# openai/ot-gan

Hardware: AMD Instinct MI355X
Metric: OT-GAN train images/sec (CIFAR-10 32x32, bs=256/GPU) (higher is better)
Workload: dtype f32 (Winograd-domain GEMMs on the fp16 matrix pipe with operands split into two scaled fp16 pieces = 22 significand bits, fp32 accumulate; errors at or below the fp32 MFMA chain's)

## Files before the change

### include/otgan_layers.h

```cpp
#ifndef OTGAN_LAYERS_H
#define OTGAN_LAYERS_H

#define OTGAN_ACT_NONE 0
#define OTGAN_ACT_CRELU 1
#define OTGAN_ACT_CELU 2
#define OTGAN_ACT_ELU 3
#define OTGAN_ACT_RELU 4

typedef struct otgan_conv_desc {
  int N;
  int H, W;
  int C;
  int ldx;
  int upsample;
  int KH, KW;
  int stride;
  int Cout;
  int ldy;
  int y_coff;
  int preact;
  int list_quads;
  const float* x_amax;
  const float* dy_amax;
  int y_accumulate;
// ... 60 lines not shown
int otgan_conv2d_dgrad_pf_f32(const otgan_conv_desc* d, const float* dy, const float* w, const void* filters,
                              const float* x, const int32_t* inv, float* dx, int lddx,
                              int accumulate, void* workspace, size_t workspace_bytes, void* stream);

int otgan_conv2d_wgrad_f32(const otgan_conv_desc* d, const float* x, const int32_t* cmap,
                           const float* dy, float* dw, void* workspace, size_t workspace_bytes,
                           void* stream);

int otgan_weightnorm_fwd_f32(const float* V, const float* g, int K, int Cout, float* w,
                             float* wT, float* inv_norm, void* stream);
int otgan_weightnorm_fwd_amax_f32(const float* V, const float* g, int K, int Cout, float* w, float* wT,
                                  float* inv_norm, float* w_amax, void* stream);
int otgan_weightnorm_bwd_f32(const float* V, const float* g, const float* inv_norm,
                             const float* dw, int K, int Cout, float* dV, float* dg,
                             float* scratch, void* stream);

#define OTGAN_WN_MAX_LAYERS 16
typedef struct otgan_wn_fwd_layer {
  const float* V;
  const float* g;
  float* w;
  float* wT;
  float* inv;
  int K;
} otgan_wn_fwd_layer;
typedef struct otgan_wn_part {
  const float* p;
  const int32_t* perm;
  int nrows;
  int rstride;
// ... 28 lines not shown
int otgan_feature_head_bwd_amax_f32(const float* x, const float* f, const float* norm, const float* df, int N, int HW,
                                    int C, float* dx, float* dx_amax, void* stream);

int otgan_adam_step_f32(float* p, const float* grad, float* v, float* mg, long n, double lr,
                        double mom1, double mom2, double t, void* stream);
#define OTGAN_ADAM_MAX_SEGMENTS 32
int otgan_adam_step_gather_f32(float* p, const float* const* grads, const long* offsets, int nseg, float* v, float* mg,
                               double lr, double mom1, double mom2, double t, float* ema_shadow, double ema_decay,
                               void* stream);
void otgan_adam_coefficients(double mom1, double mom2, double t, float* out2);
int otgan_adam_step_coef_f32(float* p, const float* grad, float* v, float* mg, long n, double lr,
                             double mom1, double mom2, double t, const float* coef_dev, void* stream);
int otgan_adam_step_gather_coef_f32(float* p, const float* const* grads, const long* offsets, int nseg, float* v, float* mg,
                                    double lr, double mom1, double mom2, double t, const float* coef_dev, float* ema_shadow,
                                    double ema_decay, void* stream);
#define OTGAN_COPY2D_MAX_SEGMENTS 64
int otgan_copy2d_batched_f32(const float* const* src, float* const* dst, const int* rows, const int* cols,
                             const long* src_ld, const long* dst_ld, int nseg, void* stream);
#define OTGAN_GATHER3D_MAX_SEGMENTS 32
int otgan_gather3d_batched_f32(const float* const* src, float* const* dst, const int* n0, int n1, int n2,
                               const long* src_s0, const long* src_s1, const long* dst_s0, const long* dst_s1,
                               int base1, const int* map1_dev, float* amax_out, int nseg, void* stream);
int otgan_adamax_step_f32(float* p, const float* grad, float* v, float* mg, long n, double lr,
                          double mom1, double mom2, void* stream);
int otgan_nesterov_step_f32(float* p, const float* grad, float* v, long n, double lr, double mom1,
                            void* stream);
int otgan_ema_update_f32(float* shadow, const float* p, long n, double decay, void* stream);

typedef struct otgan_incep_conv_desc {
  int N, H, W;
// ... 40 lines not shown
```

### ot-gan_amd/_lib_layers.py

```python
import ctypes

c_fp = ctypes.c_void_p
c_int, c_long, c_float, c_size_t = ctypes.c_int, ctypes.c_long, ctypes.c_float, ctypes.c_size_t
c_double = ctypes.c_double


class ConvDesc(ctypes.Structure):
    _fields_ = [("N", c_int), ("H", c_int), ("W", c_int), ("C", c_int), ("ldx", c_int),
                ("upsample", c_int), ("KH", c_int), ("KW", c_int), ("stride", c_int),
                ("Cout", c_int), ("ldy", c_int), ("y_coff", c_int), ("preact", c_int),
                ("list_quads", c_int), ("x_amax", ctypes.c_void_p), ("dy_amax", ctypes.c_void_p),
                ("y_accumulate", c_int), ("x_operand", ctypes.c_void_p),
                ("y_amax_out", ctypes.c_void_p), ("dx_amax_out", ctypes.c_void_p), ("w_amax", ctypes.c_void_p),
                ("x_amax_count", c_int), ("list_width", c_int),
                ("glu_out", ctypes.c_void_p), ("glu_amax_out", ctypes.c_void_p), ("dy_amax_count", c_int)]


P_DESC = ctypes.POINTER(ConvDesc)


class IncepConvDesc(ctypes.Structure):
    _fields_ = [("N", c_int), ("H", c_int), ("W", c_int), ("C", c_int), ("ldx", c_int), ("KH", c_int), ("KW", c_int),
                ("stride_h", c_int), ("stride_w", c_int), ("same", c_int), ("Cout", c_int), ("ldy", c_int),
                ("y_coff", c_int), ("relu", c_int)]
# ... 5 lines not shown
                ("y_coff", c_int)]


INCEP_POOL_MAX, INCEP_POOL_AVG = 0, 1


class Dense16BwdPair(ctypes.Structure):
    _fields_ = [("w", ctypes.c_void_p), ("fwd_filters", ctypes.c_void_p), ("filters", ctypes.c_void_p),
                ("nslices_src", c_int), ("slice_index", c_int), ("pair_index", c_int)]


class WnFwdLayer(ctypes.Structure):
    _fields_ = [("V", c_fp), ("g", c_fp), ("w", c_fp), ("wT", c_fp), ("inv", c_fp), ("K", c_int)]


class WnPart(ctypes.Structure):
    _fields_ = [("p", c_fp), ("perm", c_fp), ("nrows", c_int), ("rstride", c_int)]


class WnBwdLayer(ctypes.Structure):
    _fields_ = [("V", c_fp), ("g", c_fp), ("inv", c_fp), ("dV", c_fp), ("dg", c_fp), ("Ceff", c_int), ("taps", c_int),
                ("part", WnPart * 3)]


SIGNATURES = {
    "otgan_conv2d_workspace_bytes": (c_size_t, [P_DESC, c_int]),
    "otgan_conv2d_operand_bytes": (c_size_t, [P_DESC]),
    "otgan_conv2d_glu_fused": (c_int, [P_DESC]),
    "otgan_absmax_f32": (c_int, [c_fp, c_long, c_int, c_long, c_fp, c_fp]),
    "otgan_conv2d_amax_fused": (c_int, [P_DESC, c_int]),
# ... 8 lines not shown
    "otgan_dense16_prepare_filters_f32": (c_int, [c_fp, c_fp, c_fp, c_int, c_fp]),
    "otgan_dense16_h2_ok": (c_int, [P_DESC]),
    "otgan_dense16_chain_fwd_f32": (c_int, [c_int, c_int, c_int, c_int, c_fp, c_int, c_fp, c_fp, c_fp]),
    "otgan_dense16_chain_bwd_f32": (c_int, [c_int, c_int, c_int, c_int, c_fp, c_int, c_fp, c_int, c_fp, c_fp, c_fp, c_fp]),
    "otgan_dense16_bwd_filter_bytes": (c_size_t, [c_int]),
    "otgan_dense16_prepare_bwd_filters_f32": (c_int, [c_fp, c_int, c_fp, c_int, c_fp]),
    "otgan_dense16_bwd_slice_f32": (c_int, [c_int, c_int, c_int, c_int, c_fp, c_int, c_fp, c_fp, c_int, c_fp, c_fp, c_int,
                                            c_fp, c_int, c_fp, c_fp]),
    "otgan_conv2d_prepare_filters_f32": (c_int, [P_DESC, c_int, c_fp, c_fp, c_size_t, c_fp]),
    "otgan_conv2d_fwd_pf_f32": (c_int, [P_DESC, c_fp, c_fp, c_fp, c_fp, c_fp, c_fp, c_fp, c_size_t, c_fp]),
    "otgan_conv2d_dgrad_pf_f32": (c_int, [P_DESC, c_fp, c_fp, c_fp, c_fp, c_fp, c_fp, c_int, c_int, c_fp,
                                          c_size_t, c_fp]),
    "otgan_weightnorm_fwd_f32": (c_int, [c_fp, c_fp, c_int, c_int, c_fp, c_fp, c_fp, c_fp]),
    "otgan_weightnorm_fwd_amax_f32": (c_int, [c_fp, c_fp, c_int, c_int, c_fp, c_fp, c_fp, c_fp, c_fp]),
    "otgan_weightnorm_bwd_f32": (c_int, [c_fp, c_fp, c_fp, c_fp, c_int, c_int, c_fp, c_fp, c_fp, c_fp]),
    "otgan_weightnorm_fwd_batched16_f32": (c_int, [ctypes.POINTER(WnFwdLayer), c_int, c_fp]),
    "otgan_weightnorm_bwd_batched16_f32": (c_int, [ctypes.POINTER(WnBwdLayer), c_int, c_fp]),
    "otgan_colsum_f32": (c_int, [c_fp, c_long, c_int, c_long, c_fp, c_fp, c_fp]),
    "otgan_glu_fwd_f32": (c_int, [c_fp, c_long, c_int, c_fp, c_fp]),
    "otgan_glu_bwd_f32": (c_int, [c_fp, c_fp, c_long, c_int, c_fp, c_fp]),
    "otgan_glu_fwd_amax_f32": (c_int, [c_fp, c_long, c_int, c_fp, c_fp, c_fp]),
    "otgan_glu_bwd_amax_f32": (c_int, [c_fp, c_fp, c_long, c_int, c_fp, c_fp, c_fp]),
    "otgan_feature_head_bwd_amax_f32": (c_int, [c_fp, c_fp, c_fp, c_fp, c_int, c_int, c_int, c_fp, c_fp, c_fp]),
    "otgan_tanh_fwd_f32": (c_int, [c_fp, c_long, c_fp, c_fp]),
    "otgan_tanh_bwd_f32": (c_int, [c_fp, c_fp, c_long, c_fp, c_fp]),
    "otgan_feature_head_fwd_f32": (c_int, [c_fp, c_int, c_int, c_int, c_fp, c_fp, c_fp]),
    "otgan_feature_head_bwd_f32": (c_int, [c_fp, c_fp, c_fp, c_fp, c_int, c_int, c_int, c_fp, c_fp]),
    "otgan_adam_step_f32": (c_int, [c_fp, c_fp, c_fp, c_fp, c_long, c_double, c_double, c_double,
                                    c_double, c_fp]),
    "otgan_adam_step_gather_f32": (c_int, [c_fp, c_fp, c_fp, c_int, c_fp, c_fp, c_double, c_double, c_double, c_double,
# ... 24 lines not shown
```

### ot-gan_amd/csrc/pointwise.hip

```cpp
#include "common.h"
#include "../../include/otgan.h"

namespace {

constexpr int kChunks = 256;

inline int grid_for(long n, int per_thread = 4) {
  long b = ceil_div_l(n, 256L * per_thread);
  if (b > 4096) b = 4096;
  if (b < 1) b = 1;
  return (int)b;
}

template <int OP>
__global__ __launch_bounds__(256) void colreduce_kernel(const float* __restrict__ a,
                                                        const float* __restrict__ b, long rows,
                                                        int cols, long lda,
                                                        float* __restrict__ partial) {
  const int lane = threadIdx.x & 63, wave = threadIdx.x >> 6;
  const int c = blockIdx.x * 64 + lane;
  const int chunk = blockIdx.y;
  const long per = ceil_div_l(rows, (long)gridDim.y);
  const long r0 = chunk * per;
  long r1 = r0 + per;
// ... 62 lines not shown
  __shared__ float4 red[16][17];
  red[rsub][cq] = s;
  __syncthreads();
  if (threadIdx.x < 16 && c < cols) {
    float4 t = make_float4(0.f, 0.f, 0.f, 0.f);
#pragma unroll
    for (int k = 0; k < 16; ++k) {
      const float4 v = red[k][threadIdx.x];
      t.x += v.x; t.y += v.y; t.z += v.z; t.w += v.w;
    }
    const int cc = blockIdx.x * 64 + 4 * threadIdx.x;
    *reinterpret_cast<float4*>(partial + (long)chunk * cols + cc) = t;
  }
}

template <int OP>
int colreduce(const float* a, const float* b, long rows, int cols, long lda, float* partial,
              int* nchunk_out, hipStream_t s) {
  const int colblocks = ceil_div(cols, 64);
  long nchunk = ceil_div(1024, colblocks);
  if (nchunk > kChunks) nchunk = kChunks;
  if (nchunk > ceil_div_l(rows, 64)) nchunk = ceil_div_l(rows, 64);
  if (nchunk < 1) nchunk = 1;
  dim3 grid(colblocks, (int)nchunk);
  const bool vec = (cols % 4 == 0) && (lda % 4 == 0) && ((reinterpret_cast<uintptr_t>(a) & 15) == 0) &&
                   (!b || (reinterpret_cast<uintptr_t>(b) & 15) == 0) &&
                   ((reinterpret_cast<uintptr_t>(partial) & 15) == 0);
  if (vec) hipLaunchKernelGGL(colreduce4_kernel<OP>, grid, dim3(256), 0, s, a, b, rows, cols, lda, partial);
  else hipLaunchKernelGGL(colreduce_kernel<OP>, grid, dim3(256), 0, s, a, b, rows, cols, lda, partial);
  *nchunk_out = (int)nchunk;
  OTGAN_CHECK_LAUNCH("colreduce");
  return OTGAN_OK;
}

__global__ __launch_bounds__(256) void weightnorm_apply_kernel(const float* __restrict__ V,
                                                               const float* __restrict__ g,
                                                               const float* __restrict__ inv,
                                                               int K, int Cout,
// ... 15 lines not shown
    tile[ty + 8 * i][tx] = v;
    const unsigned b = amax_bits(v);
    mb = b > mb ? b : mb;
  }
  if (wT) {
    __syncthreads();
#pragma unroll
    for (int i = 0; i < 4; ++i) {
      const int c = c0 + ty + 8 * i, k = k0 + tx;
      if (k < K && c < Cout) wT[(long)c * K + k] = tile[tx][ty + 8 * i];
    }
  }
  if (rec) amax_commit(rec, mb);
}

__global__ void weightnorm_bwd_kernel(const float* __restrict__ V, const float* __restrict__ g,
                                      const float* __restrict__ inv, const float* __restrict__ dw,
                                      const float* __restrict__ dot, long total, int Cout,
                                      float* __restrict__ dV) {
  for (long i = (long)blockIdx.x * blockDim.x + threadIdx.x; i < total;
       i += (long)gridDim.x * blockDim.x) {
    const int c = (int)(i % Cout);
    const float iv = inv[c];
    dV[i] = g[c] * iv * (dw[i] - V[i] * dot[c] * iv * iv);
  }
}
__global__ __launch_bounds__(256) void wn_dot_finish_kernel(const float* __restrict__ partial, int nchunk, int cols,
                                                            const float* __restrict__ inv, float* __restrict__ dot,
                                                            float* __restrict__ dg) {
  const int lane = threadIdx.x & 63, part = threadIdx.x >> 6;
  const int c = blockIdx.x * 64 + lane;
  float s = 0.f;
  if (c < cols)
    for (int k = part; k < nchunk; k += 4) s += partial[(long)k * cols + c];
  __shared__ float red[4][64];
  red[part][lane] = s;
  __syncthreads();
  if (part == 0 && c < cols) {
    const float t = (red[0][lane] + red[1][lane]) + (red[2][lane] + red[3][lane]);
    dot[c] = t;
    dg[c] = t * inv[c];
  }
}
__global__ void weightnorm_dg_kernel(const float* __restrict__ dot, const float* __restrict__ inv,
                                     int Cout, float* __restrict__ dg) {
  const int c = blockIdx.x * blockDim.x + threadIdx.x;
  if (c < Cout) dg[c] = dot[c] * inv[c];
}

constexpr int kWnThreads = 512, kWnRowLanes = kWnThreads / 4;
inline bool aligned16(const void* p) { return (reinterpret_cast<uintptr_t>(p) & 15) == 0; }
struct WnFwdArgs {
  otgan_wn_fwd_layer l[OTGAN_WN_MAX_LAYERS];
};
struct WnBwdArgs {
  otgan_wn_bwd_layer l[OTGAN_WN_MAX_LAYERS];
// ... 487 lines not shown
                                   float* __restrict__ sh, float decay, float omd, const float* __restrict__ coef) {
  if (coef) {
    c1 = coef[0];
    c2 = coef[1];
  }
  const int seg = blockIdx.y;
  const long base = segs.off[seg], n = segs.off[seg + 1] - base;
  const float* __restrict__ g = segs.g[seg];
  for (long i = (long)blockIdx.x * blockDim.x + threadIdx.x; i < n; i += (long)gridDim.x * blockDim.x) {
    const long j = base + i;
    const float pn = adam_elem(p[j], g[i], v, mg, j, lr, mom1, om1, mom2, om2, c1, c2);
    p[j] = pn;
    if (sh) sh[j] = ema_elem(sh[j], pn, decay, omd);
  }
}
__global__ void ema_kernel(float* __restrict__ sh, const float* __restrict__ p, long n, float decay,
                           float omd) {
  for (long i = (long)blockIdx.x * blockDim.x + threadIdx.x; i < n; i += (long)gridDim.x * blockDim.x)
    sh[i] = ema_elem(sh[i], p[i], decay, omd);
}

}

extern "C" {

int otgan_weightnorm_fwd_amax_f32(const float* V, const float* g, int K, int Cout, float* w, float* wT,
                                  float* inv_norm, float* w_amax, void* stream) {
  OTGAN_CHECK_ARG(V && g && w && inv_norm && K > 0 && Cout > 0, "bad arguments");
  hipStream_t s = (hipStream_t)stream;
  ProfScope ps(OTGAN_PROF_POINTWISE, 0.0, 4.0 * 3 * (double)K * Cout, s);
// ... 10 lines not shown
}
int otgan_weightnorm_fwd_f32(const float* V, const float* g, int K, int Cout, float* w, float* wT, float* inv_norm,
                             void* stream) {
  return otgan_weightnorm_fwd_amax_f32(V, g, K, Cout, w, wT, inv_norm, nullptr, stream);
}

int otgan_weightnorm_bwd_f32(const float* V, const float* g, const float* inv_norm, const float* dw,
                             int K, int Cout, float* dV, float* dg, float* scratch, void* stream) {
  OTGAN_CHECK_ARG(V && g && inv_norm && dw && dV && dg && scratch && K > 0 && Cout > 0, "bad arguments");
  hipStream_t s = (hipStream_t)stream;
  ProfScope ps(OTGAN_PROF_POINTWISE, 0.0, 4.0 * 5 * (double)K * Cout, s);
  float* partial = dV;
  int nchunk = 0;
  int rc = colreduce<2>(dw, V, K, Cout, Cout, partial, &nchunk, s);
  if (rc) return rc;
  hipLaunchKernelGGL(wn_dot_finish_kernel, dim3(ceil_div(Cout, 64)), dim3(256), 0, s, partial, nchunk, Cout, inv_norm, scratch, dg);
  const long total = (long)K * Cout;
  hipLaunchKernelGGL(weightnorm_bwd_kernel, dim3(grid_for(total)), dim3(256), 0, s, V, g, inv_norm, dw,
                     scratch, total, Cout, dV);
  OTGAN_CHECK_LAUNCH("weightnorm bwd");
  return OTGAN_OK;
}

int otgan_weightnorm_fwd_batched16_f32(const otgan_wn_fwd_layer* layers, int n_layers, void* stream) {
  OTGAN_CHECK_ARG(layers && n_layers > 0, "bad arguments");
  hipStream_t s = (hipStream_t)stream;
  double bytes = 0.0;
  for (int i = 0; i < n_layers; ++i) {
    const otgan_wn_fwd_layer& l = layers[i];
    OTGAN_CHECK_ARG(l.V && l.g && l.w && l.inv && l.K > 0, "layer %d: null pointer or empty", i);
    OTGAN_CHECK_ARG(aligned16(l.V) && aligned16(l.g) && aligned16(l.w) && aligned16(l.inv), "layer %d: 16-byte alignment", i);
    bytes += 4.0 * 4 * (double)l.K * 16;
  }
  ProfScope ps(OTGAN_PROF_POINTWISE, 0.0, bytes, s);
  for (int i0 = 0; i0 < n_layers; i0 += OTGAN_WN_MAX_LAYERS) {
// ... 182 lines not shown
    segs.g[i] = grads[i];
    segs.off[i] = offsets[i];
    if (offsets[i + 1] - offsets[i] > longest) longest = offsets[i + 1] - offsets[i];
  }
  segs.off[nseg] = offsets[nseg];
  const long n = offsets[nseg] - offsets[0];
  ProfScope ps(OTGAN_PROF_POINTWISE, 0.0, 4.0 * (ema_shadow ? 9 : 7) * (double)n, s);
  float c[2] = {1.f, 1.f};
  if (!coef_dev) otgan_adam_coefficients(mom1, mom2, t, c);
  hipLaunchKernelGGL(adam_gather_kernel, dim3(grid_for(longest), nseg), dim3(256), 0, s, p, segs, v, mg, (float)lr,
                     (float)mom1, (float)(1.0 - mom1), (float)mom2, (float)(1.0 - mom2), c[0], c[1], ema_shadow,
                     (float)ema_decay, (float)(1.0 - ema_decay), coef_dev);
  OTGAN_CHECK_LAUNCH("adam (gathered gradients)");
  return OTGAN_OK;
}
int otgan_adamax_step_f32(float* p, const float* grad, float* v, float* mg, long n, double lr,
                          double mom1, double mom2, void* stream) {
  OTGAN_CHECK_ARG(p && grad && mg && n > 0 && (mom1 <= 0.0 || v), "bad arguments");
  hipLaunchKernelGGL(adamax_kernel, dim3(grid_for(n)), dim3(256), 0, (hipStream_t)stream, p, grad, v,
                     mg, n, (float)lr, (float)mom1, (float)(1.0 - mom1), (float)mom2);
  OTGAN_CHECK_LAUNCH("adamax");
  return OTGAN_OK;
}
int otgan_nesterov_step_f32(float* p, const float* grad, float* v, long n, double lr, double mom1,
                            void* stream) {
  OTGAN_CHECK_ARG(p && grad && v && n > 0, "bad arguments");
  hipLaunchKernelGGL(nesterov_kernel, dim3(grid_for(n)), dim3(256), 0, (hipStream_t)stream, p, grad,
                     v, n, (float)lr, (float)mom1, (float)(1.0 + mom1));
  OTGAN_CHECK_LAUNCH("nesterov");
  return OTGAN_OK;
// ... 11 lines not shown
```

### ot-gan_amd/ops.py

```python
import ctypes
import os
import sys
import weakref
from collections import OrderedDict

import torch

from . import _lib
from ._lib_layers import ConvDesc, WnBwdLayer, WnFwdLayer

ACT = {None: 0, "none": 0, "crelu": 1, "celu": 2, "elu": 3, "relu": 4}
DOUBLED = (1, 2)

_ws = {}


class _NullCtx:
    def __enter__(self):
        return None

    def __exit__(self, *exc):
        return False


# ... 149 lines not shown
    return w, wT, inv


def weightnorm_bwd(V2d, g, inv, dw):
    K, Cout = V2d.shape
    dV = torch.empty_like(V2d)
    dg = torch.empty_like(g)
    scratch = torch.empty(Cout, dtype=V2d.dtype, device=V2d.device)
    _lib.check(_lib.lib().otgan_weightnorm_bwd_f32(V2d.data_ptr(), g.data_ptr(), inv.data_ptr(),
                                                   dw.data_ptr(), K, Cout, dV.data_ptr(),
                                                   dg.data_ptr(), scratch.data_ptr(),
                                                   _lib.stream_ptr()), "weightnorm_bwd")
    return dV, dg


def colsum(a2d_ptr, rows, cols, lda, device):
    out = torch.empty(cols, dtype=torch.float32, device=device)
    scratch = torch.empty(256 * cols, dtype=torch.float32, device=device)
    _lib.check(_lib.lib().otgan_colsum_f32(a2d_ptr, rows, cols, lda, out.data_ptr(),
                                           scratch.data_ptr(), _lib.stream_ptr()), "colsum")
    return out


_LAUNCH_POINTERS = ("x_amax", "dy_amax", "w_amax", "y_amax_out", "dx_amax_out", "glu_out", "glu_amax_out", "x_operand")
_LAUNCH_INTS = ("ldy", "y_accumulate")


def launch_desc(desc, **fields):
    d = ConvDesc.from_buffer_copy(desc)
    for name, v in fields.items():
# ... 162 lines not shown
                                        dy.data_ptr(), dw.data_ptr(), ws.data_ptr(), ws.numel(),
                                        _lib.stream_ptr()), "conv2d_wgrad")


def fold_weights(desc, w):
    nfold = _lib.lib().otgan_conv2d_folded_weight_elems(ctypes.byref(desc))
    weff = torch.empty(nfold, dtype=w.dtype, device=w.device)
    weffT = torch.empty(nfold, dtype=w.dtype, device=w.device)
    _lib.check(_lib.lib().otgan_conv2d_fold_weights_f32(ctypes.byref(desc), w.data_ptr(), weff.data_ptr(),
                                                        weffT.data_ptr(), _lib.stream_ptr()), "fold_weights")
    return weff, weffT


SIDE_STREAM = None
_SIDE_SEEN = set()


def join_side_stream(tensors=()):
    _SIDE_SEEN.clear()
    if SIDE_STREAM is None:
        return
    cur = torch.cuda.current_stream()
    cur.wait_stream(SIDE_STREAM)
    for t in tensors:
        if t is not None and t.is_cuda:
            t.record_stream(cur)


_PENDING_GLU = [None]


def _drop_unclaimed_glu():
    ref = _PENDING_GLU[0]
    if ref is not None:
        t = ref()
        if t is not None:
            take(t, "glu", remove=True)
        _PENDING_GLU[0] = None


SIGN_TRACE = None
# ... 114 lines not shown
            conv_dgrad_raw(desc, dy, w, x, ctx.inv, dx, x.shape[3], False, filt["bwd"], dx_amax_out=dx_rec)
            if dx_rec is not None:
                tag_amax(dx, dx_rec)
        need_w = ctx.needs_input_grad[1] or ctx.needs_input_grad[2]
        need_b = ctx.has_b and ctx.needs_input_grad[3]
        side = SIDE_STREAM if (need_w or need_b) else None
        if side is not None:
            side.wait_stream(torch.cuda.current_stream())
            for t in (dy, x, ctx.x_op, dy_rec, ctx.x_rec):
                if t is not None:
                    t.record_stream(side)
        with (torch.cuda.stream(side) if side is not None else _NULL_CTX):
            if need_w:
                dw = torch.empty_like(V2d)
                conv_wgrad_raw(desc, x, ctx.cmap, dy, dw)
                dV2d, dg = weightnorm_bwd(V2d, g, inv_norm, dw)
                dV = dV2d.view(ctx.vshape)
            if need_b:
                db = colsum_of(dy)
                if db is None:
                    rows = dy.numel() // dy.shape[-1]
                    db = colsum(dy.data_ptr(), rows, dy.shape[-1], ld, dy.device)
        if side is not None:
            key = V2d.untyped_storage().data_ptr() + V2d.storage_offset()
            if key in _SIDE_SEEN:
                torch.cuda.current_stream().wait_stream(side)
            _SIDE_SEEN.add(key)
        return dx, dV, dg, db, None, None, None, None, None, None


def conv2d_op(x, V, g, b, stride=1, upsample=False, preact=0, segs=None, glu_hint=False, grow=0):
    return Conv2dFunction.apply(x, V, g, b, int(stride), bool(upsample), int(preact),
# ... 821 lines not shown


def adam_coefficients(mom1, mom2, t):
    out = (ctypes.c_float * 2)()
    _lib.lib().otgan_adam_coefficients(float(mom1), float(mom2), float(t), ctypes.cast(out, ctypes.c_void_p))
    return float(out[0]), float(out[1])


def adam_step_gather(p_flat, grads, offsets, v, mg, lr, mom1, mom2, t, ema_shadow=None, ema_decay=0.0, coef=None):
    n = len(grads)
    bump_weights_epoch(p_flat)
    if ema_shadow is not None:
        bump_weights_epoch(ema_shadow)
    gp = (ctypes.c_void_p * n)(*[g.data_ptr() for g in grads])
    off = (ctypes.c_long * (n + 1))(*offsets)
    _lib.check(_lib.lib().otgan_adam_step_gather_coef_f32(p_flat.data_ptr(), ctypes.cast(gp, ctypes.c_void_p),
                                                          ctypes.cast(off, ctypes.c_void_p), n, _lib.ptr(v), mg.data_ptr(),
                                                          float(lr), float(mom1), float(mom2), float(t), _lib.ptr(coef),
                                                          _lib.ptr(ema_shadow), float(ema_decay), _lib.stream_ptr()),
               "adam_step_gather")


COPY2D_MAX_SEGMENTS = 64


def copy2d_batched(segs):
    for i0 in range(0, len(segs), COPY2D_MAX_SEGMENTS):
        part = segs[i0:i0 + COPY2D_MAX_SEGMENTS]
        n = len(part)
        src = (ctypes.c_void_p * n)(*[q[0] for q in part])
# ... 82 lines not shown
```

### ot-gan_amd/trainer.py

```python
import importlib
import os

import torch

from . import parallel
from .utils import matching, nn


def _lib_prof_on():
    from . import _lib
    return _lib.prof_enabled()


class _frozen:

    def __init__(self, params):
        self.params = [p for p in params if p.requires_grad]

    def __enter__(self):
        for p in self.params:
            p.requires_grad_(False)

    def __exit__(self, *exc):
        for p in self.params:
# ... 95 lines not shown
        overlap = self.collectives and self.collectives_mode == "overlapped"
        self.disc_buckets = parallel.GradBuckets(self.disc_params) if overlap else None
        self.gen_buckets = parallel.GradBuckets(self.gen_params) if overlap else None
        self.gen_optimizer = mk[args.optimizer](self.gen_params, **kw)
        self.disc_optimizer = mk[args.optimizer](self.disc_params, **kw)
        self.ema_fused = self.gen_optimizer.fuse_ema(self.ema)
        self.step_counter = 0
        self.last = {}
        import collections
        self._max_ahead = 2
        self._step_ends, self._free_events = collections.deque(), []
        self.timers = None
        self._d_weights_in_graph = False
        on = side_ok
        self.fork_real_pass = self.fork_wgrad = on
        self._side_stream = torch.cuda.Stream(device=device) if on else None
        env = os.environ.get("OTGAN_STEP_GRAPH")
        asked = getattr(args, "step_graph", None)
        want = (env == "1") if env in ("0", "1") else (args.model == "densenet" if asked is None else bool(asked))
        self.graphs = GraphedSteps(self) if (want and not self.collectives and self.world == 1) else None

    def enable_timers(self, on=True):
        self.timers = {} if on else None
        if on and self.graphs is not None:
            self.graphs.drop("region timers need the eager step")
            self.graphs = None

    def _timed(self, name):
        if self.timers is None:
            return _NO_REGION
# ... 81 lines not shown

    def step(self, x_data, noise=None, apply_updates=True):
        assert x_data.shape[0] == self.nb
        period = self.args.nr_gen_per_disc + 1
        phase = self.step_counter % period
        kind = "disc" if phase == 0 else "gen"
        self._throttle()
        if self.graphs is not None and noise is None and apply_updates:
            done = self.graphs.run(x_data, phase)
            if done is not None:
                self.last = done
                self._mark_step_end()
                return self.last
        from . import ops
        ops.SIDE_STREAM = self._side_stream if self.fork_wgrad else None
        try:
            dist, ent, grads = self._step_body(x_data, kind, noise, apply_updates)
        finally:
            ops.SIDE_STREAM = None
        self._mark_step_end()
        self._d_weights_in_graph = False
        self.step_counter += 1
        self.last = {"kind": kind, "distance": dist, "entropy": ent}
        if not apply_updates:
            self.last["grads"] = grads
        return self.last

    def _throttle(self):
        if self._max_ahead > 0 and len(self._step_ends) >= self._max_ahead:
            ev = self._step_ends.popleft()
            ev.synchronize()
            self._free_events.append(ev)

    def _mark_step_end(self):
        if self._max_ahead > 0:
            ev = self._free_events.pop() if self._free_events else torch.cuda.Event()
            ev.record()
            self._step_ends.append(ev)
            if len(self._step_ends) > self._max_ahead:
                self._free_events.append(self._step_ends.popleft())

    def _optimise(self, opt, grads, lr, critic):
        opt(grads, lr=lr)
        if not critic and not self.ema_fused:
            self.maintain_averages()

    def _backward(self, outputs, params, grad_outputs):
        from . import ops
        grads = torch.autograd.grad(outputs, params, grad_outputs)
        if self.fork_wgrad:
            ops.join_side_stream(grads)
        return grads

    def prepare_step_graphs(self, x_data):
        if self.graphs is None:
            return 0
        period = self.args.nr_gen_per_disc + 1
        kinds = {self.graphs._kind(p) for p in range(period)}
        n = 0
        while self.graphs is not None and self.graphs.dead is None and set(self.graphs.graphs) != kinds and n < 3 * period + 2:
            self.step(x_data)
            n += 1
        return n
# ... 205 lines not shown
            if hasattr(opt, "ensure_state"):
                opt.ensure_state()
                if opt.coef_dev is None:
                    opt.coef_dev = torch.ones(2, dtype=torch.float32, device=m.device)
        self.x.copy_(x_data)
        ts = list(m.gen_params) + [m.ema.average(p) for p in m.gen_params]
        if kind == "gen1":
            ts += list(m.disc_params)
        self._bump(ts)
        saved_t = (m.gen_optimizer.t, m.disc_optimizer.t)
        ops.reset_amax_pool()
        g = torch.cuda.CUDAGraph()
        try:
            m.gen_optimizer.capturing = m.disc_optimizer.capturing = True
            ops.SIDE_STREAM = m._side_stream if m.fork_wgrad else None
            with torch.cuda.graph(g, stream=self.stream):
                try:
                    dist, ent, _ = m._step_body(self.x, "disc" if kind == "disc" else "gen")
                except BaseException:
                    if ops.SIDE_STREAM is not None:
                        torch.cuda.current_stream().wait_stream(ops.SIDE_STREAM)
                    raise
        finally:
            ops.SIDE_STREAM = None
            m.gen_optimizer.capturing = m.disc_optimizer.capturing = False
            m.gen_optimizer.t, m.disc_optimizer.t = saved_t
            ops.reset_amax_pool()
            ops.forget_side_events()
        self.graphs[kind] = (g, dist, ent)
        if kind == "gen1":
            self.critic_ops = ops.weights_in(m.disc_params[0])


def rank_log_kernel_slices(rank, world, f_gen, f_dat, fa, fb, lam):
    def halves(f):
        if torch.is_tensor(f):
            return f[:f.shape[0] // 2], f[f.shape[0] // 2:]
        return torch.cat(f[:len(f) // 2], 0), torch.cat(f[len(f) // 2:], 0)
    a2 = halves(fa)[1]
# ... 77 lines not shown
```

### ot-gan_amd/utils/nn.py

```python
import contextlib
import os
import threading
import weakref
from collections import OrderedDict

import torch

from .. import ops

_scope = threading.local()


def _stack():
    if not hasattr(_scope, "stack"):
        _scope.stack = []
    return _scope.stack


@contextlib.contextmanager
def arg_scope(funcs, **kwargs):
    _stack().append(({f.__name__ for f in funcs}, kwargs))
    try:
        yield
    finally:
# ... 337 lines not shown
    def __init__(self, params, lr, mom1, mom2):
        self.params = list(params)
        self.lr, self.mom1, self.mom2 = lr, mom1, mom2
        self.group = FlatGroup.of(self.params)
        self.state = [{}] if self.group is not None else [{} for _ in self.params]
        self.t = 1.0

    def fuse_ema(self, ema):
        return False

    def __call__(self, grads, lr=None):
        lr = self.lr if lr is None else lr
        with torch.no_grad():
            if self.group is not None and self._step_gather(list(grads), lr):
                pass
            elif self.group is not None:
                self._step(self.group.flat, self.group.flatten_like(list(grads), self.params), self.state[0], lr)
            else:
                for p, g, st in zip(self.params, grads, self.state):
                    self._step(p, g.contiguous(), st, lr)
        self.t += 1.0

    def state_dict(self):
        return {"t": self.t, "slots": [{k: (None if v is None else v.detach().cpu()) for k, v in st.items()}
                                       for st in self.state]}

    def load_state_dict(self, sd):
        self.t = float(sd["t"])
        targets = [self.group.flat] if self.group is not None else self.params
        if len(sd["slots"]) != len(self.state):
            raise ValueError("optimiser state does not match this parameter layout")
        for st, saved, p in zip(self.state, sd["slots"], targets):
            for k in [k for k in st if k not in saved]:
                del st[k]
            for k, v in saved.items():
                cur = st.get(k)
                if v is not None and cur is not None and cur.shape == v.shape and cur.dtype == v.dtype:
                    cur.copy_(v)
                else:
                    st[k] = None if v is None else v.to(p.device).clone()


    def _step_gather(self, grads, lr):
        return False


class _Adam(_Updates):
    _ema = None

    def fuse_ema(self, ema):
        flat = getattr(ema, "_flat", None)
        if self.group is None or flat is None or flat[1] is not self.group or len(self.params) > ops.ADAM_MAX_SEGMENTS:
            return False
        self._ema = ema
        return True

    def _step_gather(self, grads, lr):
        if len(self.params) > ops.ADAM_MAX_SEGMENTS:
            if self._ema is not None:
                raise RuntimeError("fused EMA needs the gathered Adam step")
            return False
        st, p = self.state[0], self.group.flat
        if not st:
# ... 63 lines not shown
```

Baseline: 30610.

## Defer weight-norm backward elementwise pass into the gathered Adam step

Instead of computing dV per layer in the backward pass, the conv backward now only computes per-channel dot products, dg and the g*inv scale. The raw weight gradient is passed along and the elementwise weight-norm backward is applied inside the gathered Adam kernel. This removes one full read/write pass over each weight gradient plus a kernel launch per layer. It adds bookkeeping that tags gradients, guards against shared variables and collectives, and only applies when the gathered Adam path is used.

```diff
diff --git a/include/otgan_layers.h b/include/otgan_layers.h
--- a/include/otgan_layers.h
+++ b/include/otgan_layers.h
@@ -98,6 +98,9 @@
 int otgan_weightnorm_bwd_f32(const float* V, const float* g, const float* inv_norm,
                              const float* dw, int K, int Cout, float* dV, float* dg,
                              float* scratch, void* stream);
+size_t otgan_weightnorm_bwd_partial_floats(int K, int Cout);
+int otgan_weightnorm_bwd_dots_f32(const float* V, const float* g, const float* inv_norm, const float* dw, int K, int Cout,
+                                  float* dot, float* dg, float* s, float* partial, void* stream);
 
 #define OTGAN_WN_MAX_LAYERS 16
 typedef struct otgan_wn_fwd_layer {
@@ -156,6 +159,15 @@
 int otgan_adam_step_gather_coef_f32(float* p, const float* const* grads, const long* offsets, int nseg, float* v, float* mg,
                                     double lr, double mom1, double mom2, double t, const float* coef_dev, float* ema_shadow,
                                     double ema_decay, void* stream);
+typedef struct otgan_adam_wn {
+  const float* dot;
+  const float* inv;
+  const float* s;
+  int Cout;
+} otgan_adam_wn;
+int otgan_adam_step_gather_wn_coef_f32(float* p, const float* const* grads, const otgan_adam_wn* wn, const long* offsets,
+                                       int nseg, float* v, float* mg, double lr, double mom1, double mom2, double t,
+                                       const float* coef_dev, float* ema_shadow, double ema_decay, void* stream);
 #define OTGAN_COPY2D_MAX_SEGMENTS 64
 int otgan_copy2d_batched_f32(const float* const* src, float* const* dst, const int* rows, const int* cols,
                              const long* src_ld, const long* dst_ld, int nseg, void* stream);
diff --git a/ot-gan_amd/_lib_layers.py b/ot-gan_amd/_lib_layers.py
--- a/ot-gan_amd/_lib_layers.py
+++ b/ot-gan_amd/_lib_layers.py
@@ -43,6 +43,10 @@
     _fields_ = [("V", c_fp), ("g", c_fp), ("w", c_fp), ("wT", c_fp), ("inv", c_fp), ("K", c_int)]
 
 
+class AdamWn(ctypes.Structure):
+    _fields_ = [("dot", c_fp), ("inv", c_fp), ("s", c_fp), ("Cout", c_int)]
+
+
 class WnPart(ctypes.Structure):
     _fields_ = [("p", c_fp), ("perm", c_fp), ("nrows", c_int), ("rstride", c_int)]
 
@@ -81,6 +85,10 @@
     "otgan_weightnorm_fwd_f32": (c_int, [c_fp, c_fp, c_int, c_int, c_fp, c_fp, c_fp, c_fp]),
     "otgan_weightnorm_fwd_amax_f32": (c_int, [c_fp, c_fp, c_int, c_int, c_fp, c_fp, c_fp, c_fp, c_fp]),
     "otgan_weightnorm_bwd_f32": (c_int, [c_fp, c_fp, c_fp, c_fp, c_int, c_int, c_fp, c_fp, c_fp, c_fp]),
+    "otgan_weightnorm_bwd_partial_floats": (c_size_t, [c_int, c_int]),
+    "otgan_weightnorm_bwd_dots_f32": (c_int, [c_fp, c_fp, c_fp, c_fp, c_int, c_int, c_fp, c_fp, c_fp, c_fp, c_fp]),
+    "otgan_adam_step_gather_wn_coef_f32": (c_int, [c_fp, c_fp, ctypes.POINTER(AdamWn), c_fp, c_int, c_fp, c_fp, c_double,
+                                                   c_double, c_double, c_double, c_fp, c_fp, c_double, c_fp]),
     "otgan_weightnorm_fwd_batched16_f32": (c_int, [ctypes.POINTER(WnFwdLayer), c_int, c_fp]),
     "otgan_weightnorm_bwd_batched16_f32": (c_int, [ctypes.POINTER(WnBwdLayer), c_int, c_fp]),
     "otgan_colsum_f32": (c_int, [c_fp, c_long, c_int, c_long, c_fp, c_fp, c_fp]),
diff --git a/ot-gan_amd/csrc/pointwise.hip b/ot-gan_amd/csrc/pointwise.hip
--- a/ot-gan_amd/csrc/pointwise.hip
+++ b/ot-gan_amd/csrc/pointwise.hip
@@ -100,14 +100,19 @@
   }
 }
 
-template <int OP>
-int colreduce(const float* a, const float* b, long rows, int cols, long lda, float* partial,
-              int* nchunk_out, hipStream_t s) {
+inline long colreduce_chunks(long rows, int cols) {
   const int colblocks = ceil_div(cols, 64);
   long nchunk = ceil_div(1024, colblocks);
   if (nchunk > kChunks) nchunk = kChunks;
   if (nchunk > ceil_div_l(rows, 64)) nchunk = ceil_div_l(rows, 64);
   if (nchunk < 1) nchunk = 1;
+  return nchunk;
+}
+template <int OP>
+int colreduce(const float* a, const float* b, long rows, int cols, long lda, float* partial,
+              int* nchunk_out, hipStream_t s) {
+  const int colblocks = ceil_div(cols, 64);
+  const long nchunk = colreduce_chunks(rows, cols);
   dim3 grid(colblocks, (int)nchunk);
   const bool vec = (cols % 4 == 0) && (lda % 4 == 0) && ((reinterpret_cast<uintptr_t>(a) & 15) == 0) &&
                    (!b || (reinterpret_cast<uintptr_t>(b) & 15) == 0) &&
@@ -153,6 +158,9 @@
   if (rec) amax_commit(rec, mb);
 }
 
+__device__ __forceinline__ float wn_bwd_elem(float s, float iv, float dw, float V, float dot) {
+  return s * (dw - V * dot * iv * iv);
+}
 __global__ void weightnorm_bwd_kernel(const float* __restrict__ V, const float* __restrict__ g,
                                       const float* __restrict__ inv, const float* __restrict__ dw,
                                       const float* __restrict__ dot, long total, int Cout,
@@ -161,12 +169,13 @@
        i += (long)gridDim.x * blockDim.x) {
     const int c = (int)(i % Cout);
     const float iv = inv[c];
-    dV[i] = g[c] * iv * (dw[i] - V[i] * dot[c] * iv * iv);
+    dV[i] = wn_bwd_elem(g[c] * iv, iv, dw[i], V[i], dot[c]);
   }
 }
 __global__ __launch_bounds__(256) void wn_dot_finish_kernel(const float* __restrict__ partial, int nchunk, int cols,
                                                             const float* __restrict__ inv, float* __restrict__ dot,
-                                                            float* __restrict__ dg) {
+                                                            float* __restrict__ dg, const float* __restrict__ g,
+                                                            float* __restrict__ sg) {
   const int lane = threadIdx.x & 63, part = threadIdx.x >> 6;
   const int c = blockIdx.x * 64 + lane;
   float s = 0.f;
@@ -179,6 +188,7 @@
     const float t = (red[0][lane] + red[1][lane]) + (red[2][lane] + red[3][lane]);
     dot[c] = t;
     dg[c] = t * inv[c];
+    if (sg) sg[c] = g[c] * inv[c];
   }
 }
 __global__ void weightnorm_dg_kernel(const float* __restrict__ dot, const float* __restrict__ inv,
@@ -696,6 +706,51 @@
     if (sh) sh[j] = ema_elem(sh[j], pn, decay, omd);
   }
 }
+struct AdamWnSegs {
+  AdamSegs a;
+  const float* dot[OTGAN_ADAM_MAX_SEGMENTS];
+  const float* inv[OTGAN_ADAM_MAX_SEGMENTS];
+  const float* s[OTGAN_ADAM_MAX_SEGMENTS];
+  int Cout[OTGAN_ADAM_MAX_SEGMENTS];
+};
+__global__ void adam_gather_wn_kernel(float* __restrict__ p, AdamWnSegs segs, float* __restrict__ v, float* __restrict__ mg,
+                                      float lr, float mom1, float om1, float mom2, float om2, float c1, float c2,
+                                      float* __restrict__ sh, float decay, float omd, const float* __restrict__ coef) {
+  if (coef) {
+    c1 = coef[0];
+    c2 = coef[1];
+  }
+  const int seg = blockIdx.y;
+  const long base = segs.a.off[seg], n = segs.a.off[seg + 1] - base;
+  const float* __restrict__ g = segs.a.g[seg];
+  const int Cout = segs.Cout[seg];
+  const long stride = (long)gridDim.x * blockDim.x;
+  const long i0 = (long)blockIdx.x * blockDim.x + threadIdx.x;
+  if (Cout == 0) {
+    for (long i = i0; i < n; i += stride) {
+      const long j = base + i;
+      const float pn = adam_elem(p[j], g[i], v, mg, j, lr, mom1, om1, mom2, om2, c1, c2);
+      p[j] = pn;
+      if (sh) sh[j] = ema_elem(sh[j], pn, decay, omd);
+    }
+    return;
+  }
+  const float* __restrict__ dot = segs.dot[seg];
+  const float* __restrict__ inv = segs.inv[seg];
+  const float* __restrict__ s = segs.s[seg];
+  int c = (int)(i0 % Cout);
+  const int dc = (int)(stride % Cout);
+  for (long i = i0; i < n; i += stride) {
+    const long j = base + i;
+    const float po = p[j];
+    const float gi = wn_bwd_elem(s[c], inv[c], g[i], po, dot[c]);
+    const float pn = adam_elem(po, gi, v, mg, j, lr, mom1, om1, mom2, om2, c1, c2);
+    p[j] = pn;
+    if (sh) sh[j] = ema_elem(sh[j], pn, decay, omd);
+    c += dc;
+    if (c >= Cout) c -= Cout;
+  }
+}
 __global__ void ema_kernel(float* __restrict__ sh, const float* __restrict__ p, long n, float decay,
                            float omd) {
   for (long i = (long)blockIdx.x * blockDim.x + threadIdx.x; i < n; i += (long)gridDim.x * blockDim.x)
@@ -736,11 +791,30 @@
   int nchunk = 0;
   int rc = colreduce<2>(dw, V, K, Cout, Cout, partial, &nchunk, s);
   if (rc) return rc;
-  hipLaunchKernelGGL(wn_dot_finish_kernel, dim3(ceil_div(Cout, 64)), dim3(256), 0, s, partial, nchunk, Cout, inv_norm, scratch, dg);
+  hipLaunchKernelGGL(wn_dot_finish_kernel, dim3(ceil_div(Cout, 64)), dim3(256), 0, s, partial, nchunk, Cout, inv_norm, scratch, dg,
+                     (const float*)nullptr, (float*)nullptr);
   const long total = (long)K * Cout;
   hipLaunchKernelGGL(weightnorm_bwd_kernel, dim3(grid_for(total)), dim3(256), 0, s, V, g, inv_norm, dw,
                      scratch, total, Cout, dV);
   OTGAN_CHECK_LAUNCH("weightnorm bwd");
+  return OTGAN_OK;
+}
+
+size_t otgan_weightnorm_bwd_partial_floats(int K, int Cout) {
+  if (K <= 0 || Cout <= 0) return 0;
+  return (size_t)colreduce_chunks(K, Cout) * (size_t)Cout;
+}
+int otgan_weightnorm_bwd_dots_f32(const float* V, const float* g, const float* inv_norm, const float* dw, int K, int Cout,
+                                  float* dot, float* dg, float* sg, float* partial, void* stream) {
+  OTGAN_CHECK_ARG(V && g && inv_norm && dw && dot && dg && sg && partial && K > 0 && Cout > 0, "bad arguments");
+  hipStream_t s = (hipStream_t)stream;
+  ProfScope ps(OTGAN_PROF_POINTWISE, 0.0, 4.0 * 2 * (double)K * Cout, s);
+  int nchunk = 0;
+  int rc = colreduce<2>(dw, V, K, Cout, Cout, partial, &nchunk, s);
+  if (rc) return rc;
+  hipLaunchKernelGGL(wn_dot_finish_kernel, dim3(ceil_div(Cout, 64)), dim3(256), 0, s, partial, nchunk, Cout, inv_norm, dot, dg,
+                     g, sg);
+  OTGAN_CHECK_LAUNCH("weightnorm bwd (dots)");
   return OTGAN_OK;
 }
 
@@ -953,6 +1027,38 @@
   OTGAN_CHECK_LAUNCH("adam (gathered gradients)");
   return OTGAN_OK;
 }
+int otgan_adam_step_gather_wn_coef_f32(float* p, const float* const* grads, const otgan_adam_wn* wn, const long* offsets,
+                                       int nseg, float* v, float* mg, double lr, double mom1, double mom2, double t,
+                                       const float* coef_dev, float* ema_shadow, double ema_decay, void* stream) {
+  OTGAN_CHECK_ARG(p && grads && offsets && mg && nseg > 0 && nseg <= OTGAN_ADAM_MAX_SEGMENTS && (coef_dev || t >= 1.0) && (mom1 <= 0.0 || v),
+                  "bad arguments (at most %d segments)", OTGAN_ADAM_MAX_SEGMENTS);
+  hipStream_t s = (hipStream_t)stream;
+  AdamWnSegs segs;
+  memset(&segs, 0, sizeof(segs));
+  long longest = 0;
+  for (int i = 0; i < nseg; ++i) {
+    const long len = offsets[i + 1] - offsets[i];
+    OTGAN_CHECK_ARG(grads[i] && len > 0, "segment %d: null gradient or empty range", i);
+    segs.a.g[i] = grads[i];
+    segs.a.off[i] = offsets[i];
+    if (wn && wn[i].Cout != 0) {
+      OTGAN_CHECK_ARG(wn[i].Cout > 0 && wn[i].dot && wn[i].inv && wn[i].s && len % wn[i].Cout == 0,
+                      "segment %d: weight-norm record (null pointer, or the length is no multiple of Cout)", i);
+      segs.dot[i] = wn[i].dot; segs.inv[i] = wn[i].inv; segs.s[i] = wn[i].s; segs.Cout[i] = wn[i].Cout;
+    }
+    if (len > longest) longest = len;
+  }
+  segs.a.off[nseg] = offsets[nseg];
+  const long n = offsets[nseg] - offsets[0];
+  ProfScope ps(OTGAN_PROF_POINTWISE, 0.0, 4.0 * (ema_shadow ? 9 : 7) * (double)n, s);
+  float c[2] = {1.f, 1.f};
+  if (!coef_dev) otgan_adam_coefficients(mom1, mom2, t, c);
+  hipLaunchKernelGGL(adam_gather_wn_kernel, dim3(grid_for(longest), nseg), dim3(256), 0, s, p, segs, v, mg, (float)lr,
+                     (float)mom1, (float)(1.0 - mom1), (float)mom2, (float)(1.0 - mom2), c[0], c[1], ema_shadow,
+                     (float)ema_decay, (float)(1.0 - ema_decay), coef_dev);
+  OTGAN_CHECK_LAUNCH("adam (gathered gradients, weight-norm backward inside)");
+  return OTGAN_OK;
+}
 int otgan_adamax_step_f32(float* p, const float* grad, float* v, float* mg, long n, double lr,
                           double mom1, double mom2, void* stream) {
   OTGAN_CHECK_ARG(p && grad && mg && n > 0 && (mom1 <= 0.0 || v), "bad arguments");
diff --git a/ot-gan_amd/ops.py b/ot-gan_amd/ops.py
--- a/ot-gan_amd/ops.py
+++ b/ot-gan_amd/ops.py
@@ -7,7 +7,7 @@
 import torch
 
 from . import _lib
-from ._lib_layers import ConvDesc, WnBwdLayer, WnFwdLayer
+from ._lib_layers import AdamWn, ConvDesc, WnBwdLayer, WnFwdLayer
 
 ACT = {None: 0, "none": 0, "crelu": 1, "celu": 2, "elu": 3, "relu": 4}
 DOUBLED = (1, 2)
@@ -187,6 +187,21 @@
     return dV, dg
 
 
+WN_DEFERRED = False
+
+
+def weightnorm_bwd_dots(V2d, g, inv, dw):
+    K, Cout = V2d.shape
+    L = _lib.lib()
+    dg = torch.empty_like(g)
+    cols = torch.empty((2, Cout), dtype=V2d.dtype, device=V2d.device)
+    partial = torch.empty(L.otgan_weightnorm_bwd_partial_floats(K, Cout), dtype=V2d.dtype, device=V2d.device)
+    _lib.check(L.otgan_weightnorm_bwd_dots_f32(V2d.data_ptr(), g.data_ptr(), inv.data_ptr(), dw.data_ptr(), K, Cout,
+                                               cols[0].data_ptr(), dg.data_ptr(), cols[1].data_ptr(), partial.data_ptr(),
+                                               _lib.stream_ptr()), "weightnorm_bwd_dots")
+    return dg, {"V_ptr": V2d.data_ptr(), "Cout": Cout, "dot": cols[0], "s": cols[1], "inv": inv}
+
+
 def colsum(a2d_ptr, rows, cols, lda, device):
     out = torch.empty(cols, dtype=torch.float32, device=device)
     scratch = torch.empty(256 * cols, dtype=torch.float32, device=device)
@@ -379,10 +394,12 @@
 
 SIDE_STREAM = None
 _SIDE_SEEN = set()
+WN_SEEN = set()
 
 
 def join_side_stream(tensors=()):
     _SIDE_SEEN.clear()
+    WN_SEEN.clear()
     if SIDE_STREAM is None:
         return
     cur = torch.cuda.current_stream()
@@ -390,6 +407,9 @@
     for t in tensors:
         if t is not None and t.is_cuda:
             t.record_stream(cur)
+            rec = take(t, "wn")
+            if rec is not None:
+                rec["dot"].record_stream(cur)
 
 
 _PENDING_GLU = [None]
@@ -534,8 +554,17 @@
             if need_w:
                 dw = torch.empty_like(V2d)
                 conv_wgrad_raw(desc, x, ctx.cmap, dy, dw)
-                dV2d, dg = weightnorm_bwd(V2d, g, inv_norm, dw)
-                dV = dV2d.view(ctx.vshape)
+                if WN_DEFERRED:
+                    key = V2d.data_ptr()
+                    if key in WN_SEEN:
+                        raise RuntimeError("deferred weight-norm backward: a variable used twice in one graph would have its "
+                                           "raw weight gradients summed")
+                    WN_SEEN.add(key)
+                    dg, rec = weightnorm_bwd_dots(V2d, g, inv_norm, dw)
+                    dV = leave(dw.view(ctx.vshape), "wn", rec)
+                else:
+                    dV2d, dg = weightnorm_bwd(V2d, g, inv_norm, dw)
+                    dV = dV2d.view(ctx.vshape)
             if need_b:
                 db = colsum_of(dy)
                 if db is None:
@@ -1387,6 +1416,21 @@
         bump_weights_epoch(ema_shadow)
     gp = (ctypes.c_void_p * n)(*[g.data_ptr() for g in grads])
     off = (ctypes.c_long * (n + 1))(*offsets)
+    recs = [take(g, "wn") for g in grads]
+    if any(r is not None for r in recs):
+        wn = (AdamWn * n)()
+        for i, r in enumerate(recs):
+            if r is None:
+                continue
+            if r["V_ptr"] != p_flat.data_ptr() + 4 * offsets[i]:
+                raise ValueError("deferred weight-norm backward: the gradient's variable is not this segment of the buffer")
+            wn[i].dot, wn[i].inv, wn[i].s, wn[i].Cout = r["dot"].data_ptr(), r["inv"].data_ptr(), r["s"].data_ptr(), r["Cout"]
+        _lib.check(_lib.lib().otgan_adam_step_gather_wn_coef_f32(p_flat.data_ptr(), ctypes.cast(gp, ctypes.c_void_p), wn,
+                                                                 ctypes.cast(off, ctypes.c_void_p), n, _lib.ptr(v),
+                                                                 mg.data_ptr(), float(lr), float(mom1), float(mom2), float(t),
+                                                                 _lib.ptr(coef), _lib.ptr(ema_shadow), float(ema_decay),
+                                                                 _lib.stream_ptr()), "adam_step_gather (weight norm inside)")
+        return
     _lib.check(_lib.lib().otgan_adam_step_gather_coef_f32(p_flat.data_ptr(), ctypes.cast(gp, ctypes.c_void_p),
                                                           ctypes.cast(off, ctypes.c_void_p), n, _lib.ptr(v), mg.data_ptr(),
                                                           float(lr), float(mom1), float(mom2), float(t), _lib.ptr(coef),
diff --git a/ot-gan_amd/trainer.py b/ot-gan_amd/trainer.py
--- a/ot-gan_amd/trainer.py
+++ b/ot-gan_amd/trainer.py
@@ -133,6 +133,7 @@
         self._d_weights_in_graph = False
         on = side_ok
         self.fork_real_pass = self.fork_wgrad = on
+        self.wn_deferred = True
         self._side_stream = torch.cuda.Stream(device=device) if on else None
         env = os.environ.get("OTGAN_STEP_GRAPH")
         asked = getattr(args, "step_graph", None)
@@ -244,10 +245,12 @@
                 return self.last
         from . import ops
         ops.SIDE_STREAM = self._side_stream if self.fork_wgrad else None
+        ops.WN_DEFERRED = self._defers_weightnorm(kind, apply_updates)
         try:
             dist, ent, grads = self._step_body(x_data, kind, noise, apply_updates)
         finally:
             ops.SIDE_STREAM = None
+            ops.WN_DEFERRED = False
         self._mark_step_end()
         self._d_weights_in_graph = False
         self.step_counter += 1
@@ -270,6 +273,12 @@
             if len(self._step_ends) > self._max_ahead:
                 self._free_events.append(self._step_ends.popleft())
 
+    def _defers_weightnorm(self, kind, apply_updates=True):
+        opt = self.disc_optimizer if kind == "disc" else self.gen_optimizer
+        observed = "_optimise" in self.__dict__
+        return bool(self.wn_deferred and apply_updates and not self.collectives and not observed and
+                    opt.takes_raw_weight_gradients())
+
     def _optimise(self, opt, grads, lr, critic):
         opt(grads, lr=lr)
         if not critic and not self.ema_fused:
@@ -277,6 +286,7 @@
 
     def _backward(self, outputs, params, grad_outputs):
         from . import ops
+        ops.WN_SEEN.clear()
         grads = torch.autograd.grad(outputs, params, grad_outputs)
         if self.fork_wgrad:
             ops.join_side_stream(grads)
@@ -512,6 +522,7 @@
         try:
             m.gen_optimizer.capturing = m.disc_optimizer.capturing = True
             ops.SIDE_STREAM = m._side_stream if m.fork_wgrad else None
+            ops.WN_DEFERRED = m._defers_weightnorm("disc" if kind == "disc" else "gen")
             with torch.cuda.graph(g, stream=self.stream):
                 try:
                     dist, ent, _ = m._step_body(self.x, "disc" if kind == "disc" else "gen")
@@ -521,6 +532,7 @@
                     raise
         finally:
             ops.SIDE_STREAM = None
+            ops.WN_DEFERRED = False
             m.gen_optimizer.capturing = m.disc_optimizer.capturing = False
             m.gen_optimizer.t, m.disc_optimizer.t = saved_t
             ops.reset_amax_pool()
diff --git a/ot-gan_amd/utils/nn.py b/ot-gan_amd/utils/nn.py
--- a/ot-gan_amd/utils/nn.py
+++ b/ot-gan_amd/utils/nn.py
@@ -375,6 +375,8 @@
         with torch.no_grad():
             if self.group is not None and self._step_gather(list(grads), lr):
                 pass
+            elif any(ops.take(g, "wn") is not None for g in grads):
+                raise RuntimeError("raw weight gradients (ops.WN_DEFERRED) need the gathered Adam step")
             elif self.group is not None:
                 self._step(self.group.flat, self.group.flatten_like(list(grads), self.params), self.state[0], lr)
             else:
@@ -405,9 +407,15 @@
     def _step_gather(self, grads, lr):
         return False
 
+    def takes_raw_weight_gradients(self):
+        return False
+
 
 class _Adam(_Updates):
     _ema = None
+
+    def takes_raw_weight_gradients(self):
+        return self.group is not None and len(self.params) <= ops.ADAM_MAX_SEGMENTS
 
     def fuse_ema(self, ema):
         flat = getattr(ema, "_flat", None)
```

Result: no change. 30470 (-0.5%).
